# haoy945/DeMF

Hardware: AMD Instinct MI355X
Metric: DeMF fusion fwd+bwd scenes/sec at 20k pts + 530x730 RGB (higher is better)
Workload: dtype f32; 1 GPU; BASELINE configs[2]: full DeMF fusion hot path fwd+loss+bwd+allreduce+AdamW, 8 scenes/GPU x (20000 pts, 800x1120 -> 4-level 256-ch pyramid), 256 queries, H=8 L=4 P=2, fp32; compute_mode=f32, scenes_per_gpu=8, parallelism=dp1, cloud=uniform

## Files before the change

### demf_amd/_ffi.py

```python
import ctypes
import os

_HERE = os.path.dirname(os.path.abspath(__file__))
LIB_PATH = os.environ.get("DEMF_LIB_PATH") or os.path.join(_HERE, "lib", "libdemf_hip.so")

_c_int = ctypes.c_int
_c_float = ctypes.c_float
_ptr = ctypes.c_void_p

SIGNATURES = {
    "demf_stream_create_cu_masked": [_ptr, _c_int, _c_int, _ptr],
    "demf_spin_us": [_c_int, _ptr],
    "demf_conv_nhwc_f32": [_c_int] * 9 + [_ptr, _ptr, _c_int, _ptr, _ptr, _c_int, _c_int, _ptr, _ptr],
    "demf_conv_stem7_nhwc4_f32": [_c_int] * 4 + [_ptr, _ptr, _c_int, _ptr, _c_int, _ptr, _ptr],
    "demf_maxpool3x3s2_nhwc_f32": [_c_int] * 4 + [_ptr, _ptr, _ptr],
    "demf_nchw3_to_nhwc4_f32": [_c_int] * 3 + [_ptr, _ptr, _ptr],
    "demf_groupnorm_nhwc_f32": [_c_int] * 4 + [_c_float, _ptr, _ptr, _ptr, _ptr, _ptr, ctypes.c_longlong, _ptr],
    "demf_fps_f32": [_c_int, _c_int, _c_int, _ptr, _ptr, _ptr, _ptr],
    "demf_fps_ws_f32": [_c_int, _c_int, _c_int, _ptr, _ptr, ctypes.c_longlong, _ptr, _ptr],
    "demf_ball_query_f32": [_c_int, _c_int, _c_int, _c_float, _c_float, _c_int, _ptr, _ptr,
                            _ptr, _ptr],
    "demf_ball_query_grid_ws": [_c_int, _c_int, _ptr, _ptr],
    "demf_ball_query_grid_f32": [_c_int, _c_int, _c_int, _c_float, _c_int] + [_ptr] * 6,
    "demf_group_points_fwd": [_c_int] * 5 + [_ptr] * 4,
# ... 60 lines not shown
    "demf_multi_add": [_c_int, _ptr, _c_int, _ptr],
    "demf_multi_add_sumsq": [_c_int, _ptr, _c_int, _ptr, _ptr],
    "demf_scalars_accum": [_c_int, _ptr, _ptr, _c_float, _ptr],
    "demf_mlp_gemm_fwd": [_c_int] * 4 + [_ptr] * 6,
    "demf_mlp_gemm_fwd_pool": [_c_int] * 4 + [_ptr] * 5 + [_c_int] + [_ptr] * 5,
    "demf_mlp_gemm_fwd_bn": [_c_int] * 4 + [_ptr] * 7 + [_c_float, _c_float] + [_ptr] * 7,
    "demf_mlp_gemm_fwd_pool_bn": [_c_int] * 4 + [_ptr] * 5 + [_c_int] + [_ptr] * 6 + [_c_float, _c_float] + [_ptr] * 7,
    "demf_mlp_gemm_fwd_bn_st": [_c_int] * 4 + [_ptr] * 7 + [_c_float, _c_float] + [_ptr] * 6 + [_c_int, _ptr],
    "demf_mlp_gemm_fwd_pool_bn_st": [_c_int] * 4 + [_ptr] * 5 + [_c_int] + [_ptr] * 4 + [_c_float, _c_float] + [_ptr] * 6 + [_c_int, _ptr],
    "demf_pool_select": [_c_int] * 2 + [_ptr] * 9,
    "demf_pool_select_slot0": [_c_int] * 2 + [_ptr] * 7,
    "demf_mlp_first_stats": [_c_int] * 2 + [_ptr] * 5 + [_c_float, _c_float] + [_ptr] * 7,
    "demf_mlp_gemm_fwd_bn_x4": [_c_int] * 2 + [_ptr] * 8 + [_c_float, _c_float] + [_ptr] * 7,
    "demf_mlp_bwd_fused_x4": [_c_int] * 3 + [_ptr] * 11,
    "demf_mlp_bwd_pool": [_c_int] * 4 + [_ptr] * 17,
    "demf_mlp_bwd_pool_ws": [_c_int, _ptr],
    "demf_bn_finalize": [_c_int, ctypes.c_longlong] + [_ptr] * 3 + [_c_float, _c_float] + [_ptr] * 7,
    "demf_l2norm_rows_fwd": [_c_int] * 2 + [_ptr] * 4,
    "demf_l2norm_rows_bwd": [_c_int] * 2 + [_ptr] * 5,
    "demf_vote_combine_fwd": [_c_int] * 2 + [_ptr] * 7,
    "demf_vote_combine_bwd": [_c_int] * 2 + [_ptr] * 7,
    "demf_bnrelu_maxpool_fwd": [_c_int] * 3 + [_ptr] * 5,
    "demf_bn_bwd_reduce": [_c_int] * 3 + [_ptr] * 9,
    "demf_bn_bwd_vectors": [_c_int, ctypes.c_longlong] + [_ptr] * 8,
    "demf_mlp_gemm_bwd_dx": [_c_int] * 4 + [_ptr] * 3 + [_c_int] + [_ptr] * 5,
    "demf_mlp_gemm_bwd_dx_first": [_c_int] * 3 + [_ptr] * 10,
    "demf_mlp_first_finish": [_c_int, ctypes.c_longlong] + [_ptr] * 7,
    "demf_mlp_gemm_bwd_dx_red": [_c_int] * 4 + [_ptr] * 3 + [_c_int] + [_ptr] * 9,
    "demf_mlp_gemm_bwd_dx_w": [_c_int] * 4 + [_ptr] * 3 + [_c_int] + [_ptr] * 5,
    "demf_mlp_bwd_fused": [_c_int] * 3 + [_ptr] * 3 + [_c_int] + [_ptr] * 15 + [_c_int, _ptr],
    "demf_mlp_bwd_fused_cols": [_c_int] * 5 + [_ptr] * 3 + [_c_int] + [_ptr] * 14,
    "demf_mlp_bwd_fused_wide": [_c_int] * 3 + [_ptr] * 3 + [_c_int] + [_ptr] * 14,
    "demf_mlp_last_form": [],
    "demf_switch_at": [_c_int, _ptr, _ptr, _ptr],
    "demf_mlp_gemm_bwd_dx_red_v": [_c_int] * 4 + [_ptr] * 3 + [_c_int] + [_ptr] * 13,
    "demf_bn_bwd_reduce_vectors": [_c_int] * 3 + [_ptr] * 11 + [_c_int, _ptr],
    "demf_mlp_gemm_bwd_dw": [_c_int] * 4 + [_ptr] * 3 + [_c_int] + [_ptr] * 6,
    "demf_mlp_gemm_bwd_dw_ld": [_c_int] * 4 + [_ptr] * 3 + [_c_int] + [_ptr] * 5 + [_c_int, _ptr],
    "demf_head_loss_fwd": [_c_int] * 3 + [_ptr] * 14,
    "demf_head_loss_bwd": [_c_int] * 3 + [_ptr] * 17,
    "demf_ca_head_loss_fwd": [_c_int] * 3 + [_ptr] * 12,
    "demf_ca_head_loss_bwd": [_c_int] * 3 + [_ptr] * 16,
    "demf_vote_loss": [_c_int] * 4 + [_c_float] + [_ptr] * 10,
    "demf_vote_loss_fwd": [_c_int] * 4 + [_c_float] + [_ptr] * 8,
    "demf_msda_fwd_f32": [_c_int] * 7 + [_ptr] * 7,
    "demf_msda_bwd_f32": [_c_int] * 7 + [_ptr] * 10,
    "demf_msda_fwd_bf16": [_c_int] * 7 + [_ptr] * 7,
    "demf_msda_bwd_bf16": [_c_int] * 7 + [_ptr] * 10,
    "demf_gemm_f32": [_ptr, _ptr],
    "demf_gemm_group_f32": [_ptr, _c_int, _ptr],
    "demf_set_compute_dtype": [_c_int],
    "demf_set_f16_terms": [_c_int],
    "demf_get_compute_dtype": [],
    "demf_ctx_push": [_ptr],
    "demf_ctx_pop": [],
    "demf_gemm_f32_ctx": [_ptr] * 3,
    "demf_gemm_group_f32_ctx": [_ptr, _ptr, _c_int, _ptr],
    "demf_mlp_gemm_fwd_ctx": [_ptr] + [_c_int] * 4 + [_ptr] * 6,
    "demf_multi_copy": [_c_int, _ptr, _c_int, _ptr],
    "demf_zero_f32": [ctypes.c_longlong, _ptr, _ptr],
    "demf_add_dropout_ln_fwd": [_c_int] * 2 + [_ptr] * 4 + [_c_float] * 2 + [_ptr, _c_int] + [_ptr] * 4,
    "demf_add_dropout_ln_bwd": [_c_int] * 2 + [_ptr] * 5 + [_c_float, _ptr, _c_int, _ptr, _c_int] + [_ptr] * 4,
    "demf_attn_core_fwd": [_c_int] * 4 + [_ptr, _c_float, _c_float, _ptr, _c_int] + [_ptr] * 5,
    "demf_attn_core_bwd": [_c_int] * 4 + [_ptr] * 4 + [_c_float, _c_float, _ptr, _c_int] + [_ptr] * 2,
    "demf_softmax_dropout_fwd": [_c_int] * 2 + [_ptr, _c_float, _ptr, _c_int] + [_ptr] * 3,
    "demf_softmax_dropout_bwd": [_c_int] * 2 + [_ptr, _c_float, _ptr, _c_int] + [_ptr] * 2,
# ... 76 lines not shown
```

### demf_amd/csrc/mlp_bwd.hip

```cpp
#include "common.h"
#include "bn_fin.h"
#include "wide_map.h"

namespace demf {

using f32x16 = float __attribute__((ext_vector_type(16)));
using bf16x8 = __bf16 __attribute__((ext_vector_type(8)));
using bf16x4 = __bf16 __attribute__((ext_vector_type(4)));
using bf16x2 = __bf16 __attribute__((ext_vector_type(2)));

struct FusedBwdArgs {
  int R, N, K, ns;
  const float* Yl;
  const float* G;
  const float* dP;
  const int* arg;
  const float* vec;
  const float* Xp;
  const float* pss;
  const float* pmi;
  const float* W;
  float* dX;
  float* dW;
  double* g12;
  const float* fX;
  double* fsum;
  BnVecFin vfin;
  int ldk, ldw, fld, fc0;
  const float* W0;
  int dbg;
  int nchunk;
};

template <int P>
__device__ __forceinline__ void split_planes(float x, __bf16 (&o)[P]) {
  if constexpr (P == 2) {
    const _Float16 h = (_Float16)x;
    o[0] = __builtin_bit_cast(__bf16, h);
    o[1] = __builtin_bit_cast(__bf16, (_Float16)(x - (float)h));
    return;
  }
  o[0] = (__bf16)x;
  if constexpr (P == 3) {
    const float r = x - (float)o[0];
    o[1] = (__bf16)r;
    o[2] = (__bf16)(r - (float)o[1]);
  }
}

using f32x2 = float __attribute__((ext_vector_type(2)));
template <int P>
__device__ __forceinline__ void split_pair(float a, float b, unsigned (&o)[P]) {
  if constexpr (P == 2) {
    split2_f16(a, b, o[0], o[1]);
    return;
  }
  const f32x2 x = {a, b};
  const bf16x2 h = __builtin_convertvector(x, bf16x2);
  o[0] = __builtin_bit_cast(unsigned, h);
  if constexpr (P == 3) {
    const f32x2 r = x - __builtin_convertvector(h, f32x2);
    const bf16x2 m = __builtin_convertvector(r, bf16x2);
    o[1] = __builtin_bit_cast(unsigned, m);
    const f32x2 l = r - __builtin_convertvector(m, f32x2);
    o[2] = __builtin_bit_cast(unsigned, __builtin_convertvector(l, bf16x2));
// ... 19 lines not shown
    acc = __builtin_amdgcn_mfma_f32_32x32x16_bf16(a[0], b[0], acc, 0, 0, 0);
  } else {
    acc = __builtin_amdgcn_mfma_f32_32x32x16_bf16(a[0], b[0], acc, 0, 0, 0);
  }
}

__device__ __forceinline__ float f16_scale_for(float m) {
  int e = (int)((__builtin_bit_cast(unsigned, m) >> 23) & 0xff) - 127;
  e = 3 - e;
  e = e < -100 ? -100 : (e > 100 ? 100 : e);
  return __builtin_bit_cast(float, (unsigned)(e + 127) << 23);
}

template <int CW, bool B16>
__device__ __forceinline__ auto load_row(const float* __restrict__ base, size_t elem) {
  using vecT = float __attribute__((ext_vector_type(CW)));
  if constexpr (!B16) {
    return *reinterpret_cast<const vecT*>(base + elem);
  } else {
    const __bf16* b = reinterpret_cast<const __bf16*>(base) + elem;
    vecT v;
    if constexpr (CW == 4) {
      const uint2 u = *reinterpret_cast<const uint2*>(b);
      v[0] = __builtin_bit_cast(float, u.x << 16); v[1] = __builtin_bit_cast(float, u.x & 0xffff0000u);
      v[2] = __builtin_bit_cast(float, u.y << 16); v[3] = __builtin_bit_cast(float, u.y & 0xffff0000u);
    } else {
      const unsigned u = *reinterpret_cast<const unsigned*>(b);
      v[0] = __builtin_bit_cast(float, u << 16); v[1] = __builtin_bit_cast(float, u & 0xffff0000u);
    }
    return v;
  }
}

template <int NTN, int KT, int KG, bool SPARSE, int CM, int EPI, int ST = 0, bool WIDE = false>
__global__ __launch_bounds__(64 * NTN * KG, 512 / (64 * NTN * KG)) void mlp_bwd_fused_kernel(FusedBwdArgs p) {
  static_assert(!WIDE || (EPI == 0 && ST == 0), "WIDE: RED epilogue, fp32 rows");
  constexpr bool XB = (ST & 1) != 0, YB = (ST & 2) != 0;
  constexpr bool XR = (ST & 4) != 0;
  static_assert(!XR || (EPI == 1 && !XB), "recomputed rows: FIRST epilogue, no storage type");
  constexpr int P = CM == 2 ? 3 : (CM == 3 ? 2 : 1);
  constexpr bool H2 = CM == 3;
  constexpr int N = NTN * 32, K = KT * 32;
  constexpr int NW = NTN * KG;
  constexpr int NT = 64 * NW;
  constexpr int RS = 32;
  constexpr int KTW = KT / KG;
  constexpr int CW = 4 / KG;
  constexpr int LPB = 32 / CW;
  constexpr int QK = K / 4;
  constexpr int ER = NT / QK;
  constexpr int NH = NW / KT;
  constexpr int SL = NTN / NH;
  constexpr int CR = 16 / NH;
  static_assert(NW % KT == 0 && NH >= 1 && NTN % NH == 0 && SL >= 1, "dX wave map");
  static_assert(KG >= 1 && KTW >= 1 && KT % KG == 0 && (NW == 4 || NW == 8), "unsupported shape");
  static_assert(2 * ER == RS && 4 * (K / 64) == NW, "epilogue / staging maps");
  static_assert(EPI == 0 || (!SPARSE), "FIRST is a dense layer");
  constexpr int REGB = P * 2 * 2048;
  constexpr int XATB = P * K * 64;
  extern __shared__ __attribute__((aligned(16))) char smem[];
  char* s_reg = smem;
  char* s_xat = s_reg + NTN * REGB;
  float* s_dx = reinterpret_cast<float*>(s_xat + XATB);
  float* s_vy = s_dx + RS * K;
  float* s_px = s_vy + 5 * N;
  float* s_w0 = s_px + 4 * K;
  float* s_mx = s_w0 + 4 * K;
  const int tid = threadIdx.x, lane = tid & 63;
  const int wave = __builtin_amdgcn_readfirstlane(tid >> 6);
  const int lr = lane & 31, lh = lane >> 5;
  const int nt = wave % NTN, kg = wave / NTN;
  int w_fc0 = 0, w_slab0 = 0, w_step = 0;
  if constexpr (WIDE) {
    const WideBlock wb = wide_block((int)blockIdx.x, p.nchunk, (int)gridDim.x / p.nchunk);
    w_fc0 = __builtin_amdgcn_readfirstlane(wb.chunk * (KT * 32));
// ... 310 lines not shown
          }
          if constexpr (EPI == 0) {
            if constexpr (YB) {
              unsigned o0[1], o1[1];
              split_pair<1>(dx.x, dx.y, o0);
              split_pair<1>(dx.z, dx.w, o1);
              *reinterpret_cast<uint2*>(reinterpret_cast<__bf16*>(p.dX) + (size_t)row * p.ldk + 4 * e_cq) = make_uint2(o0[0], o1[0]);
            } else {
              *reinterpret_cast<float4*>(FB_PTR(p.dX) + (size_t)row * p.ldk + 4 * e_cq) = dx;
            }
          } else {
            const float4 x = *reinterpret_cast<const float4*>(p.fX + (size_t)row * 4);
            const float yv[4] = {y.x, y.y, y.z, y.w};
#pragma unroll
            for (int c = 0; c < 4; ++c) {
              fs[c][0] = __builtin_fmaf(dz[c], x.x, fs[c][0]);
              fs[c][1] = __builtin_fmaf(dz[c], x.y, fs[c][1]);
              fs[c][2] = __builtin_fmaf(dz[c], x.z, fs[c][2]);
              fs[c][3] = __builtin_fmaf(dz[c], x.w, fs[c][3]);
              fs[c][4] = __builtin_fmaf(yv[c], x.x, fs[c][4]);
              fs[c][5] = __builtin_fmaf(yv[c], x.y, fs[c][5]);
              fs[c][6] = __builtin_fmaf(yv[c], x.z, fs[c][6]);
              fs[c][7] = __builtin_fmaf(yv[c], x.w, fs[c][7]);
            }
            if (e_cq == 0) { fcx[0] += x.x; fcx[1] += x.y; fcx[2] += x.z; fcx[3] += x.w; }
          }
        }
      }
    }
  }

  __syncthreads();
  float* s_red = reinterpret_cast<float*>(smem);
  if (!(p.dbg & 1)) {
    const float inv = H2 ? 1.0f / sc_cur : 1.0f;
#pragma unroll
    for (int kk = 0; kk < KTW; ++kk)
#pragma unroll
      for (int r = 0; r < 16; ++r) {
        const int n = 32 * nt + (r & 3) + 8 * (r >> 2) + 4 * lh;
        const int k = 32 * (kg * KTW + kk) + lr;
        atomicAdd(FB_PTR(p.dW) + (size_t)n * p.ldw + k, H2 ? dwacc[kk][r] * inv : dwacc[kk][r]);
      }
  }
  constexpr int NV = EPI == 1 ? 8 + 32 + 4 : 8;
  float v[NV];
#pragma unroll
  for (int c = 0; c < 4; ++c) { v[c] = es1[c]; v[4 + c] = es2[c]; }
  if constexpr (EPI == 1) {
#pragma unroll
    for (int c = 0; c < 4; ++c)
#pragma unroll
      for (int q = 0; q < 8; ++q) v[8 + c * 8 + q] = fs[c][q];
#pragma unroll
    for (int c = 0; c < 4; ++c) v[40 + c] = fcx[c];
  }
#pragma unroll
  for (int i = 0; i < NV; ++i)
#pragma unroll
    for (int m = QK; m < 64; m <<= 1) v[i] += __shfl_xor(v[i], m);
  if (lane < QK) {
#pragma unroll
    for (int i = 0; i < NV; ++i) s_red[(wave * QK + lane) * NV + i] = v[i];
  }
  __syncthreads();
  for (int i = tid; i < QK * NV; i += NT) {
    const int cq = i / NV, q = i % NV;
    float t = 0.f;
#pragma unroll
    for (int w = 0; w < NW; ++w) t += s_red[(w * QK + cq) * NV + q];
    if (q < 8) {
      const int col = 4 * cq + (q & 3);
      if constexpr (EPI == 0) atomicAdd(p.g12 + (q >> 2) * p.fld + FB_FC0 + col, (double)t);
      else atomicAdd(p.fsum + (q >> 2) * K + col, (double)t);
    } else if (q < 40) {
      const int c = (q - 8) >> 3, s = (q - 8) & 7, col = 4 * cq + c;
      atomicAdd(p.fsum + (s < 4 ? 2 * K + col * 4 + s : 6 * K + col * 4 + (s - 4)), (double)t);
    } else if (cq == 0) {
      atomicAdd(p.fsum + 10 * K + (q - 40), (double)t);
    }
  }
  if constexpr (EPI == 0) {
    if (p.vfin.ticket != nullptr) {
      __shared__ int s_last;
      sync_drained();
      if (tid == 0) s_last = last_workgroup(p.vfin.ticket, (int)gridDim.x, (int)blockIdx.x);
      __syncthreads();
      if (s_last) bn_vec_finalize(p.vfin, p.fld, WIDE ? 0 : p.fc0, WIDE ? p.fld : K, p.g12, tid, NT);
    }
  }
#undef FB_FC0
#undef FB_STEP
#undef FB_PTR
}

struct PoolBwdArgs {
  int R, ns;
  const float* Xp;
  const float* pss;
  const float* pmi;
  const float* W;
  const float* vec;
  const float* dP;
  const int* arg;
  const float* yraw;
  float* dX;
  float* part;
  double* g12;
  BnVecFin vfin;
  int dbg;
};
constexpr int PB_N = 128, PB_K = 64, PB_RS = 64;
constexpr int PB_NACC = PB_N * PB_K;
constexpr int PB_LDA = PB_K + 4;
constexpr int PB_LDM = PB_K + 4;
// ... 356 lines not shown
    __shared__ int s_last;
    sync_drained();
    if (tid == 0) s_last = last_workgroup(p.vfin.ticket, (int)gridDim.x, (int)blockIdx.x);
    __syncthreads();
    if (s_last) bn_vec_finalize(p.vfin, K, 0, K, p.g12, tid, NT);
  }
}

__global__ __launch_bounds__(256) void pool_bwd_finish_k(int nslots, const float* __restrict__ part,
                                                         float* __restrict__ dW) {
  __shared__ float s_f[8][32];
  const int el = threadIdx.x & 31, sl = threadIdx.x >> 5;
  const int e = blockIdx.x * 32 + el;
  float t[8] = {0.f, 0.f, 0.f, 0.f, 0.f, 0.f, 0.f, 0.f};
  if (e < PB_NACC) {
    int s = sl;
    for (; s + 56 < nslots; s += 64) {
#pragma unroll
      for (int u = 0; u < 8; ++u) t[u] += part[(size_t)(s + 8 * u) * PB_NACC + e];
    }
    for (; s < nslots; s += 8) t[0] += part[(size_t)s * PB_NACC + e];
  }
  s_f[sl][el] = ((t[0] + t[1]) + (t[2] + t[3])) + ((t[4] + t[5]) + (t[6] + t[7]));
  __syncthreads();
  if (sl == 0 && e < PB_NACC)
    dW[e] = ((s_f[0][el] + s_f[1][el]) + (s_f[2][el] + s_f[3][el])) + ((s_f[4][el] + s_f[5][el]) + (s_f[6][el] + s_f[7][el]));
}

static int vectors_without_ticket(const BnVecFin& vf, int K, double* g12, demf_stream_t stream) {
  if (vf.gamma == nullptr || vf.ticket != nullptr) return DEMF_OK;
  return demf_bn_bwd_vectors(K, (long long)vf.count, g12, vf.gamma, vf.ss, vf.mi, vf.vec, vf.dgamma, vf.dbeta, stream);
}

template <int NTN, int KT, int KG, bool SPARSE, int CM, int EPI, int ST = 0, bool WIDE = false>
static int launch_fused(const FusedBwdArgs& a, hipStream_t s) {
  constexpr int P = CM == 2 ? 3 : (CM == 3 ? 2 : 1);
  constexpr int N = NTN * 32, K = KT * 32, NW = NTN * KG;
  const size_t bytes = (size_t)NTN * P * 2 * 2048 + (size_t)P * K * 64 + sizeof(float) * (32 * K + 5 * N + 4 * K + 4 * K + 24);
  static unsigned long long reserved = 0;
  if (!reserve_lds(reinterpret_cast<const void*>(&mlp_bwd_fused_kernel<NTN, KT, KG, SPARSE, CM, EPI, ST, WIDE>), (int)bytes,
                   &reserved)) {
    set_error("mlp_bwd_fused: cannot reserve %zu bytes of LDS", bytes);
    return DEMF_ELAUNCH;
  }
  const int nslab = (a.R + 31) / 32;
  const int cap = sw().persist_cus_bwd * (8 / NW);
  const int gx = WIDE ? a.nchunk * wide_members(nslab, a.nchunk, cap) : (nslab < cap ? nslab : cap);
  hipLaunchKernelGGL((mlp_bwd_fused_kernel<NTN, KT, KG, SPARSE, CM, EPI, ST, WIDE>), dim3(gx), dim3(64 * NW), bytes, s, a);
  return check_launch("mlp_bwd_fused");
}

}

using namespace demf;

static int fused_h2_mode() {
  return sw().f16_terms_bwd;
}
static bool fused_h2_on() { return fused_h2_mode() != 0; }

static int fused_supported(int R, int N, int K, int ns, int sparse, int first) {
  const int cm = compute_mode();
  if (cm != 1 && cm != 2) return 0;
  if (R < 1) return 0;
  if (sparse && (ns < 4 || ns % 4 != 0 || R % ns != 0)) return 0;
  if (first) return (N == 64 && K == 64 && !sparse) ? 1 : 0;
  return ((N == 128 && K == 64) || (N == 128 && K == 128) || (N == 64 && K == 64) || (N == 256 && K == 128)) ? 1 : 0;
}

extern "C" int demf_mlp_bwd_fused(int R, int N, int K, const float* G, const float* dP, const int* arg,
                                  int ns, const float* Y, const float* vec6, const float* W,
                                  const float* Yprev, const float* scale_shift_prev,
                                  const float* mean_invstd_prev, float* dX, float* dW, double* g12_prev,
                                  const float* X0, double* first_sums, const float* gamma_prev,
                                  float* vec6_prev, float* dgamma_prev, float* dbeta_prev,
                                  int store_flags, demf_stream_t stream) {
  const bool sparse = G == nullptr, first = first_sums != nullptr;
  DEMF_REQUIRE(fused_supported(R, N, K, ns, sparse, first),
               "mlp_bwd_fused: unsupported shape / mode R=%d N=%d K=%d ns=%d sparse=%d first=%d mode=%d",
               R, N, K, ns, (int)sparse, (int)first, compute_mode());
  DEMF_REQUIRE(Y && vec6 && W && Yprev && scale_shift_prev && mean_invstd_prev && dW &&
                   (G || (dP && arg)) && (first ? (X0 != nullptr) : (dX && g12_prev)),
// ... 84 lines not shown
  const bool sparse = G == nullptr;
  constexpr int Kc = 128;
  DEMF_REQUIRE(N == 256 && fused_supported(R, N, Kc, ns, sparse, 0) && Ktot > Kc && Ktot % Kc == 0 && Ktot <= 512,
               "mlp_bwd_fused_wide: unsupported shape / mode R=%d N=%d Ktot=%d ns=%d sparse=%d mode=%d",
               R, N, Ktot, ns, (int)sparse, compute_mode());
  DEMF_REQUIRE(Y && vec6 && W && Yprev && scale_shift_prev && mean_invstd_prev && dW && (G || (dP && arg)) && dX &&
                   g12_prev, "mlp_bwd_fused_wide: null pointer");
  set_last_form(DEMF_FORM_FUSED_WIDE);
  FusedBwdArgs a{};
  a.dbg = sw().bwd_dbg;
  a.R = R; a.N = N; a.K = Kc; a.ns = ns; a.Yl = Y; a.G = G; a.dP = dP; a.arg = arg; a.vec = vec6;
  a.Xp = Yprev; a.dX = dX; a.W = W; a.dW = dW;
  a.pss = scale_shift_prev; a.pmi = mean_invstd_prev; a.g12 = g12_prev;
  a.ldk = Ktot; a.ldw = Ktot; a.fld = Ktot; a.fc0 = 0; a.nchunk = Ktot / Kc;
  if (gamma_prev != nullptr) {
    DEMF_REQUIRE(vec6_prev && dgamma_prev && dbeta_prev, "mlp_bwd_fused_wide: vectors of layer l-1 need all three outputs");
    a.vfin = BnVecFin{(double)R, gamma_prev, scale_shift_prev, mean_invstd_prev, vec6_prev, dgamma_prev,
                      dbeta_prev, sched_slot()};
  }
  hipStream_t s = (hipStream_t)stream;
  const int cm = compute_mode();
  const bool h2 = f16_terms() && fused_h2_on();
  int rc;
  if (sparse) {
    rc = cm == 1 ? launch_fused<8, 4, 1, true, 1, 0, 0, true>(a, s)
                 : (h2 ? launch_fused<8, 4, 1, true, 3, 0, 0, true>(a, s) : launch_fused<8, 4, 1, true, 2, 0, 0, true>(a, s));
  } else {
    rc = cm == 1 ? launch_fused<8, 4, 1, false, 1, 0, 0, true>(a, s)
                 : (h2 ? launch_fused<8, 4, 1, false, 3, 0, 0, true>(a, s) : launch_fused<8, 4, 1, false, 2, 0, 0, true>(a, s));
  }
  return rc ? rc : vectors_without_ticket(a.vfin, Ktot, g12_prev, stream);
}

static int pool_bwd_grid(int R) {
  const int cus = sw().persist_cus_bwd;
  const int nslab = R / PB_RS;
  return nslab < cus ? (nslab > 0 ? nslab : 1) : cus;
}

extern "C" int demf_mlp_bwd_pool_ws(int R, long long* floats) {
  DEMF_REQUIRE(R >= 0 && floats, "mlp_bwd_pool_ws: bad arguments");
  *floats = (long long)pool_bwd_grid(R) * PB_NACC;
  return DEMF_OK;
}

extern "C" int demf_mlp_bwd_pool(int R, int N, int K, int ns, const float* dP, const int* arg,
                                 const float* yraw, const float* vec6, const float* W, const float* Yprev,
                                 const float* scale_shift_prev, const float* mean_invstd_prev, float* dX,
                                 float* dW, double* g12_prev, const float* gamma_prev, float* vec6_prev,
                                 float* dgamma_prev, float* dbeta_prev, float* workspace,
                                 demf_stream_t stream) {
  const int cm = compute_mode();
  DEMF_REQUIRE((cm == 1 || cm == 2) && N == PB_N && K == PB_K && ns == PB_RS && R >= ns && R % ns == 0,
               "mlp_bwd_pool: unsupported shape / mode R=%d N=%d K=%d ns=%d mode=%d", R, N, K, ns, cm);
  DEMF_REQUIRE(dP && arg && yraw && vec6 && W && Yprev && scale_shift_prev && mean_invstd_prev && dX && dW &&
                   g12_prev && workspace, "mlp_bwd_pool: null pointer");
  set_last_form(DEMF_FORM_POOL);
  PoolBwdArgs a{};
  a.R = R; a.ns = ns; a.Xp = Yprev; a.pss = scale_shift_prev; a.pmi = mean_invstd_prev; a.W = W; a.vec = vec6;
  a.dP = dP; a.arg = arg; a.yraw = yraw; a.dX = dX; a.part = workspace; a.g12 = g12_prev;
  a.dbg = sw().pb_dbg;
  if (gamma_prev != nullptr) {
    DEMF_REQUIRE(vec6_prev && dgamma_prev && dbeta_prev, "mlp_bwd_pool: vectors of layer l-1 need all three outputs");
    a.vfin = BnVecFin{(double)R, gamma_prev, scale_shift_prev, mean_invstd_prev, vec6_prev, dgamma_prev,
                      dbeta_prev, sched_slot()};
  }
// ... 49 lines not shown
```

### demf_amd/csrc/switches.h

```cpp
#pragma once

namespace demf {

#define DEMF_SWITCHES(X) \
  X(f32_native,         "DEMF_F32_NATIVE",         0,     "initial compute mode: 1 = fp32 MFMA (mode 0) instead of three bf16 terms (mode 2)") \
  X(f16_terms,          "DEMF_F16_TERMS",          1,     "initial two-fp16-term setting of mode 2 (demf_set_f16_terms overrides)") \
  X(f16_terms_bwd,      "DEMF_F16_TERMS_BWD",      1,     "fused backward: 0 = three bf16 terms, 1 = two fp16 terms, 2 = also the pool form") \
  X(x3_mask,            "DEMF_X3_MASK",            7,     "mode 2 per kernel family: bit 0 forward, bit 1 dX, bit 2 weight gradient") \
  X(static_tiles,       "DEMF_STATIC_TILES",       0,     "1 = static tile schedule, no BN-finalize ticket in the GEMM") \
  X(acc_repl,           "DEMF_ACC_REPL",           1,     "replicated statistics accumulators") \
  X(acc_repl_fwd,       "DEMF_ACC_REPL_FWD",       0,     "replicated accumulators in the forward finalize") \
  X(acc_repl_red,       "DEMF_ACC_REPL_RED",       0,     "replicated accumulators in the dX reduce finalize") \
  X(gemm_grid,          "DEMF_GEMM_GRID",          512,   "block cap of the persistent shared-MLP GEMM") \
  X(persist_cus,        "DEMF_PERSIST_CUS",        240,   "blocks of the weight-resident / producer-consumer forwards") \
  X(persist_cus_bwd,    "DEMF_PERSIST_CUS_BWD",    240,   "blocks of the fused backwards; unset = DEMF_PERSIST_CUS (reported value is the effective one)") \
  X(fwd_pc,             "DEMF_FWD_PC",             1,     "producer/consumer forward (K = 128)") \
  X(fwd_pc_min_r,       "DEMF_FWD_PC_MIN_R",       16384, "fewest rows for the producer/consumer forward") \
  X(fwd_res,            "DEMF_FWD_RES",            1,     "weight-resident forward (K = 64, N = 64 / 128)") \
  X(fwd_tile,           "DEMF_FWD_TILE",           1,     "few-row tile forward") \
  X(fwd_tile_max_r,     "DEMF_FWD_TILE_MAX_R",     16384, "most rows for the tile forward") \
  X(dx_tile,            "DEMF_DX_TILE",            1,     "few-row tile dX") \
  X(dx_tile_max_r,      "DEMF_DX_TILE_MAX_R",      16384, "most rows for the tile dX") \
  X(dx_chunks,          "DEMF_DX_CHUNKS",          0,     "chunked dX reduce") \
  X(pool_halves,        "DEMF_POOL_HALVES",        0,     "1 = ns 64 pooling on two co-scheduled column halves") \
  X(pool_dyn,           "DEMF_POOL_DYN",           1,     "dynamic tile schedule in the pooling GEMM") \
  X(x3_wide_split,      "DEMF_X3_WIDE_SPLIT",      1,     "0 = wide three-term forwards on the fp32 MFMA instead of a column split") \
  X(split_target,       "DEMF_SPLIT_TARGET",       256,   "blocks the column split aims at") \
  X(no_fin,             "DEMF_NO_FIN",             0,     "1 = no in-kernel BN finalize") \
  X(bnred_ns1_dense,    "DEMF_BNRED_NS1_DENSE",    1,     "dense form of the BN-backward reduce at ns = 1") \
  X(bnred_pooled_dense, "DEMF_BNRED_POOLED_DENSE", 1,     "dense form of the BN-backward reduce on pooled rows") \
  X(bnred_rpb,          "DEMF_BNRED_RPB",          8,     "rows per thread of the replicated dense reduce") \
  X(bnred_grid,         "DEMF_BNRED_GRID",         -1,    "block cap of the dense reduce; -1 = 1024 replicated, 256 otherwise") \
  X(bnred_rev,          "DEMF_BNRED_REV",          1,     "dense reduce visits its rows last to first") \
  X(bnred_sparse_rpt,   "DEMF_BNRED_SPARSE_RPT",   8,     "rows per thread of the sparse reduce") \
  X(bnred_sparse_grid,  "DEMF_BNRED_SPARSE_GRID",  1024,  "block cap of the sparse reduce") \
  X(dw_small_r,         "DEMF_DW_SMALL_R",         65536, "weight-gradient launches of at most this many rows use 64 x 64 sub-blocks") \
  X(dw_tile,            "DEMF_DW_TILE",            0,     "weight-gradient sub-block: 12 = 64 x 128, 21 = 128 x 64, 22, 11") \
  X(dw_f32,             "DEMF_DW_F32",             0,     "bf16 mode: weight gradient on fp32 operands") \
  X(dw_grid,            "DEMF_DW_GRID",            512,   "blocks of the grouped weight-gradient launch") \
  X(dw_dyn,             "DEMF_DW_DYN",             0,     "dynamic schedule of the weight-gradient launch") \
  X(dw_dbg,             "DEMF_DW_DBG",             0,     "weight gradient: phase-skip timing experiments") \
  X(dw_trace,           "DEMF_DW_TRACE",           0,     "print the step's weight-gradient products (tools/dw_micro.py)") \
  X(bwd_dbg,            "DEMF_BWD_DBG",            0,     "fused backward: phase-skip timing experiments") \
  X(pb_dbg,             "DEMF_PB_DBG",             0,     "pool backward: phase-skip timing experiments") \
  X(gemm_small_tiles,   "DEMF_GEMM_SMALL_TILES",   1024,  "demf_gemm_f32 launches of at most this many 64 x 64 tiles use the 32 x 32 kernel") \
  X(gemm_tn3,           "DEMF_GEMM_TN3",           1,     "0 = no three-term TN GEMM") \
  X(gemm_tn_split,      "DEMF_GEMM_TN_SPLIT",      0,     "forced K split of the TN GEMM") \
  X(tn_dbg,             "DEMF_TN_DBG",             0,     "TN GEMM: phase-skip timing experiments") \
  X(ln_bwd_blocks,      "DEMF_LN_BWD_BLOCKS",      256,   "blocks of the LayerNorm backward (at least 1)") \
  X(rg_dbg,             "DEMF_RG_DBG",             0,     "row GEMM chain: phase-skip timing experiments") \
  X(rg_ln128,           "DEMF_RG_LN128",           0,     "row GEMM chain: the 128-row LayerNorm form") \
  X(rg_waves8,          "DEMF_RG_WAVES8",          0,     "row GEMM chain: the 8-wave forms") \
  X(rg_add4,            "DEMF_RG_ADD4",            0,     "row GEMM chain: the adding form on 4 waves") \
  X(rg_one,             "DEMF_RG_ONE",             0,     "row GEMM chain: non-zero = one workgroup per CU") \
  X(conv_stream64,      "DEMF_CONV_STREAM64",      1,     "streaming 1x1 convolution at K = 64") \
  X(conv_streamk,       "DEMF_CONV_STREAMK",       3,     "streaming 1x1 convolution: bit 0 K = 128, bit 1 K = 256") \
  X(conv_stream_min,    "DEMF_CONV_STREAM_MIN",    16384, "fewest rows for the streaming convolution") \
  X(conv_wg3,           "DEMF_CONV_WG3",           0,     "three-plane convolutions: three workgroups per CU") \
  X(msda_head_wgs,      "DEMF_MSDA_HEAD_WGS",      256,   "workgroups the (scene, head)-major attention aims at") \
  X(msda_raw_lanes,     "DEMF_MSDA_RAW_LANES",     0,     "non-zero = 8 lanes per query in the raw form") \
  X(msda_xcd,           "DEMF_MSDA_XCD",           0,     "XCD-aware block order") \
  X(msda_nt,            "DEMF_MSDA_NT",            1,     "non-temporal loads of the raw offsets / logits") \
  X(gf_fwd_blocks,      "DEMF_GF_FWD_BLOCKS",      1024,  "block cap of the group-first forward") \
  X(gf_bwd_blocks,      "DEMF_GF_BWD_BLOCKS",      0,     "block cap of the group-first backward (0 = its own choice)") \
  X(gf_fin,             "DEMF_GF_FIN",             1,     "0 = group-first forward without the in-kernel finalize") \
  X(gf_recompute,       "DEMF_GF_RECOMPUTE",       1,     "0 = group-first backward reads stored activations") \
  X(gf_wacc,            "DEMF_GF_WACC",            1,     "0 = group-first backward without the in-kernel weight gradient") \
  X(colsum_rows,        "DEMF_COLSUM_ROWS",        64,    "fewest rows per block of the column sum") \
  X(invert_split,       "DEMF_INVERT_SPLIT",       1,     "invert_index as five launches when the lists leave LDS; 2 = from 32 768 entries, 0 = never") \
  X(three_nn_split,     "DEMF_THREE_NN_SPLIT",     1,     "split form of three_nn") \
  X(fps_check_split,    "DEMF_FPS_CHECK_SPLIT",    1,     "two-kernel form of the FPS order check") \
  X(fps_prune,          "DEMF_FPS_PRUNE",          1,     "box-pruned FPS on large clouds") \
  X(fps_pair,           "DEMF_FPS_PAIR",           -1,    "per-pair cached maxima: -1 = above 16 slots per lane, 0 / 1 force") \
  X(fps_pair_waves,     "DEMF_FPS_PAIR_WAVES",     16,    "waves of the pair kernel (8 or 16)") \
  X(fps_waves,          "DEMF_FPS_WAVES",          16,    "waves of the pruned kernel (8 or 16)")

// ... 10 lines not shown
```

### demf_amd/csrc/wide_map.h

```cpp
#pragma once

#if defined(__HIPCC__)
#define DEMF_WM_HD __host__ __device__ __forceinline__
#else
#define DEMF_WM_HD static inline
#endif

namespace demf {

struct WideBlock {
  int chunk;
  int first;
  int stride;
};

DEMF_WM_HD int wide_members(int nslab, int nchunk, int cap) {
  int g = cap / nchunk;
  if (g > nslab) g = nslab;
  if (g < 1) g = 1;
  if (g >= 8) g -= g % 8;
  return g;
}

DEMF_WM_HD int wide_run(int gpc) { return gpc >= 8 ? 8 : gpc; }

DEMF_WM_HD WideBlock wide_block(int block, int nchunk, int gpc) {
  const int rw = wide_run(gpc);
  const int run = block / (rw * nchunk), within = block % (rw * nchunk);
  WideBlock b;
  b.chunk = within / rw;
  b.first = run * rw + within % rw;
  b.stride = gpc;
  return b;
}

}
```

### include/demf_hip.h

```cpp
#ifndef DEMF_HIP_H_
#define DEMF_HIP_H_

#include <stdint.h>

#ifdef __cplusplus
extern "C" {
#endif

typedef void* demf_stream_t;

#define DEMF_OK 0
#define DEMF_EINVAL (-1)
#define DEMF_ELAUNCH (-2)
#define DEMF_EUNSUPPORTED (-3)

#define DEMF_ABI_VERSION 2

#define DEMF_INTERNAL

int demf_version(void);
const char* demf_last_error(void);

DEMF_INTERNAL int demf_stream_create_cu_masked(const int* cus, int n, int invert, void** out);

// ... 207 lines not shown
                                 int ns, float* pmax, int* amax, const float* gamma, const float* beta,
                                 float eps, float momentum, float* running_mean, float* running_var,
                                 long long* num_batches_tracked, float* scale_shift, float* mean_invstd,
                                 const float* conv_bias, int store_flags, demf_stream_t stream);

DEMF_INTERNAL int demf_mlp_bwd_fused(int R, int N, int K, const float* G, const float* dP, const int* arg, int ns,
                       const float* Y, const float* vec6, const float* W, const float* Yprev,
                       const float* scale_shift_prev, const float* mean_invstd_prev, float* dX,
                       float* dW, double* g12_prev, const float* X0, double* first_sums,
                       const float* gamma_prev, float* vec6_prev, float* dgamma_prev, float* dbeta_prev,
                       int store_flags, demf_stream_t stream);
DEMF_INTERNAL int demf_mlp_bwd_fused_cols(int R, int N, int Ktot, int c0, int Kc, const float* G, const float* dP,
                            const int* arg, int ns, const float* Y, const float* vec6, const float* W,
                            const float* Yprev, const float* scale_shift_prev,
                            const float* mean_invstd_prev, float* dX, float* dW, double* g12_prev,
                            const float* gamma_prev, float* vec6_prev, float* dgamma_prev,
                            float* dbeta_prev, demf_stream_t stream);
DEMF_INTERNAL int demf_mlp_bwd_fused_wide(int R, int N, int Ktot, const float* G, const float* dP, const int* arg, int ns,
                            const float* Y, const float* vec6, const float* W, const float* Yprev,
                            const float* scale_shift_prev, const float* mean_invstd_prev, float* dX,
                            float* dW, double* g12_prev, const float* gamma_prev, float* vec6_prev,
                            float* dgamma_prev, float* dbeta_prev, demf_stream_t stream);

#define DEMF_FORM_NONE 0
#define DEMF_FORM_GENERIC 1
#define DEMF_FORM_TILE 2
#define DEMF_FORM_RES 3
#define DEMF_FORM_PC 4
#define DEMF_FORM_FUSED 5
#define DEMF_FORM_FUSED_COLS 6
#define DEMF_FORM_FUSED_WIDE 7
#define DEMF_FORM_POOL 8
DEMF_INTERNAL int demf_mlp_last_form(void);

DEMF_INTERNAL int demf_switch_at(int index, const char** name, int* value, int* dflt);

DEMF_INTERNAL int demf_mlp_first_stats(int R, int N0, const float* X, const float* W0, double* moments, const float* gamma,
                         const float* beta, float eps, float momentum, float* running_mean,
                         float* running_var, long long* num_batches_tracked, float* scale_shift,
                         float* mean_invstd, const float* conv_bias, demf_stream_t stream);
DEMF_INTERNAL int demf_mlp_gemm_fwd_bn_x4(int R, int N, const float* X4, const float* W0, const float* prev_scale_shift,
                            const float* Wt, float* Y, double* stats, const float* gamma, const float* beta,
                            float eps, float momentum, float* running_mean, float* running_var,
                            long long* num_batches_tracked, float* scale_shift, float* mean_invstd,
                            const float* conv_bias, demf_stream_t stream);
DEMF_INTERNAL int demf_mlp_bwd_fused_x4(int R, int N, int K, const float* G, const float* Y, const float* vec6,
                          const float* W, const float* X0, const float* W0, const float* scale_shift_prev,
                          const float* mean_invstd_prev, float* dW, double* first_sums, demf_stream_t stream);

DEMF_INTERNAL int demf_mlp_bwd_pool_ws(int R, long long* floats);
DEMF_INTERNAL int demf_mlp_bwd_pool(int R, int N, int K, int ns, const float* dP, const int* arg, const float* yraw,
                      const float* vec6, const float* W, const float* Yprev,
                      const float* scale_shift_prev, const float* mean_invstd_prev, float* dX, float* dW,
                      double* g12_prev, const float* gamma_prev, float* vec6_prev, float* dgamma_prev,
                      float* dbeta_prev, float* workspace, demf_stream_t stream);

DEMF_INTERNAL int demf_mlp_gemm_bwd_dw(int R, int N, int K, int ldx, const float* G, const float* dP,
                         const int* arg, int ns, const float* Y, const float* vec6,
                         const float* Xprev, const float* prev_scale_shift, float* dW,
                         demf_stream_t stream);
DEMF_INTERNAL int demf_mlp_gemm_bwd_dw_ld(int R, int N, int K, int ldx, const float* G, const float* dP,
                            const int* arg, int ns, const float* Y, const float* vec6,
                            const float* Xprev, const float* prev_scale_shift, float* dW, int lddw,
                            demf_stream_t stream);

typedef struct demf_dw_job {
// ... 312 lines not shown
```

Measured before the change: 1926 scenes/s.

## Fold fused-backward dW partials per same-XCD workgroup group before atomics

For fused MLP backward kernels with 128 input channels, each workgroup writes its dW partial tile to a global slot buffer. A per-group ticket picks the last-arriving workgroup of a group of (by default) 4 same-XCD workgroups, which sums the partials and issues the atomicAdds alone. This cuts global float atomics on dW by roughly the group size, at the cost of extra global stores and loads, release/acquire fences and a serial reduction tail in one workgroup per group. It also adds a switch and a debug query for ticket state.

```diff
diff --git a/demf_amd/_ffi.py b/demf_amd/_ffi.py
--- a/demf_amd/_ffi.py
+++ b/demf_amd/_ffi.py
@@ -116,6 +116,7 @@
     "demf_mlp_bwd_fused_cols": [_c_int] * 5 + [_ptr] * 3 + [_c_int] + [_ptr] * 14,
     "demf_mlp_bwd_fused_wide": [_c_int] * 3 + [_ptr] * 3 + [_c_int] + [_ptr] * 14,
     "demf_mlp_last_form": [],
+    "demf_mlp_bwd_flush_state": [_ptr, _ptr],
     "demf_switch_at": [_c_int, _ptr, _ptr, _ptr],
     "demf_mlp_gemm_bwd_dx_red_v": [_c_int] * 4 + [_ptr] * 3 + [_c_int] + [_ptr] * 13,
     "demf_bn_bwd_reduce_vectors": [_c_int] * 3 + [_ptr] * 11 + [_c_int, _ptr],
diff --git a/demf_amd/csrc/mlp_bwd.hip b/demf_amd/csrc/mlp_bwd.hip
--- a/demf_amd/csrc/mlp_bwd.hip
+++ b/demf_amd/csrc/mlp_bwd.hip
@@ -30,7 +30,12 @@
   const float* W0;
   int dbg;
   int nchunk;
+  int fgroup;
 };
+
+constexpr int FLUSH_SLOTS = 256, FLUSH_SLOT = 256 * 128, FLUSH_TICKETS = 256;
+__device__ float g_flush_slots[(size_t)FLUSH_SLOTS * FLUSH_SLOT];
+__device__ int g_flush_tickets[FLUSH_TICKETS];
 
 template <int P>
 __device__ __forceinline__ void split_planes(float x, __bf16 (&o)[P]) {
@@ -116,7 +121,7 @@
   }
 }
 
-template <int NTN, int KT, int KG, bool SPARSE, int CM, int EPI, int ST = 0, bool WIDE = false>
+template <int NTN, int KT, int KG, bool SPARSE, int CM, int EPI, int ST = 0, bool WIDE = false, bool FL = false>
 __global__ __launch_bounds__(64 * NTN * KG, 512 / (64 * NTN * KG)) void mlp_bwd_fused_kernel(FusedBwdArgs p) {
   static_assert(!WIDE || (EPI == 0 && ST == 0), "WIDE: RED epilogue, fp32 rows");
   constexpr bool XB = (ST & 1) != 0, YB = (ST & 2) != 0;
@@ -125,6 +130,7 @@
   constexpr int P = CM == 2 ? 3 : (CM == 3 ? 2 : 1);
   constexpr bool H2 = CM == 3;
   constexpr int N = NTN * 32, K = KT * 32;
+  static_assert(!FL || (EPI == 0 && ST == 0 && K == 128), "FL: RED epilogue, fp32 rows, 128 input channels");
   constexpr int NW = NTN * KG;
   constexpr int NT = 64 * NW;
   constexpr int RS = 32;
@@ -501,16 +507,59 @@
 
   __syncthreads();
   float* s_red = reinterpret_cast<float*>(smem);
-  if (!(p.dbg & 1)) {
-    const float inv = H2 ? 1.0f / sc_cur : 1.0f;
+  [[maybe_unused]] int fl_v = (int)blockIdx.x, fl_n = 0, fl_ch = 0;
+  [[maybe_unused]] FlushGroup fl_g{0, 1, 0};
+  [[maybe_unused]] float4* fl_slot0 = nullptr;
+  [[maybe_unused]] auto flush_add = [&]() {
 #pragma unroll
     for (int kk = 0; kk < KTW; ++kk)
 #pragma unroll
       for (int r = 0; r < 16; ++r) {
         const int n = 32 * nt + (r & 3) + 8 * (r >> 2) + 4 * lh;
         const int k = 32 * (kg * KTW + kk) + lr;
-        atomicAdd(FB_PTR(p.dW) + (size_t)n * p.ldw + k, H2 ? dwacc[kk][r] * inv : dwacc[kk][r]);
-      }
+        atomicAdd(FB_PTR(p.dW) + (size_t)n * p.ldw + k, dwacc[kk][r]);
+      }
+  };
+  if constexpr (!FL) {
+    if (!(p.dbg & 1)) {
+      const float inv = H2 ? 1.0f / sc_cur : 1.0f;
+#pragma unroll
+      for (int kk = 0; kk < KTW; ++kk)
+#pragma unroll
+        for (int r = 0; r < 16; ++r) {
+          const int n = 32 * nt + (r & 3) + 8 * (r >> 2) + 4 * lh;
+          const int k = 32 * (kg * KTW + kk) + lr;
+          atomicAdd(FB_PTR(p.dW) + (size_t)n * p.ldw + k, H2 ? dwacc[kk][r] * inv : dwacc[kk][r]);
+        }
+    }
+  } else if (!(p.dbg & 1)) {
+    if constexpr (H2) {
+      const float inv = 1.0f / sc_cur;
+#pragma unroll
+      for (int kk = 0; kk < KTW; ++kk)
+#pragma unroll
+        for (int r = 0; r < 16; ++r) dwacc[kk][r] *= inv;
+    }
+    fl_n = (int)gridDim.x;
+    if constexpr (WIDE) {
+      fl_n = (int)gridDim.x / p.nchunk;
+      const WideBlock wb = wide_block((int)blockIdx.x, p.nchunk, fl_n);
+      fl_v = wide_member(wb);
+      fl_ch = wb.chunk;
+    }
+    fl_g = flush_group(fl_v, fl_n, p.fgroup);
+    fl_slot0 = reinterpret_cast<float4*>(g_flush_slots) + (size_t)(fl_ch * fl_n) * (FLUSH_SLOT / 4) +
+               (size_t)(wave * KTW * 4) * 64 + lane;
+    if (fl_g.size > 1) {
+      float4* mine = fl_slot0 + (size_t)fl_v * (FLUSH_SLOT / 4);
+#pragma unroll
+      for (int kk = 0; kk < KTW; ++kk)
+#pragma unroll
+        for (int q = 0; q < 4; ++q)
+          mine[(kk * 4 + q) * 64] = make_float4(dwacc[kk][4 * q], dwacc[kk][4 * q + 1], dwacc[kk][4 * q + 2], dwacc[kk][4 * q + 3]);
+    } else {
+      flush_add();
+    }
   }
   constexpr int NV = EPI == 1 ? 8 + 32 + 4 : 8;
   float v[NV];
@@ -549,7 +598,63 @@
       atomicAdd(p.fsum + 10 * K + (q - 40), (double)t);
     }
   }
-  if constexpr (EPI == 0) {
+  if constexpr (FL) {
+    int* s_flag = reinterpret_cast<int*>(s_mx + 16);
+    const bool grouped = !(p.dbg & 1) && fl_g.size > 1;
+    sync_drained();
+    if (tid == 0) {
+      int last = 0;
+      if (grouped) {
+        if (!(p.dbg & 8)) __builtin_amdgcn_fence(__ATOMIC_RELEASE, "agent");
+        drain_vmem();
+        int* t = g_flush_tickets + fl_ch * flush_tickets(fl_n, p.fgroup) + fl_g.ticket;
+        last = __hip_atomic_fetch_add(t, 1, __ATOMIC_RELAXED, __HIP_MEMORY_SCOPE_AGENT) == fl_g.size - 1;
+        if (last) {
+          atomicExch(t, 0);
+          __builtin_amdgcn_fence(__ATOMIC_ACQUIRE, "agent");
+          drain_vmem();
+        }
+      }
+      s_flag[0] = last;
+      s_flag[1] = p.vfin.ticket != nullptr ? last_workgroup(p.vfin.ticket, (int)gridDim.x, (int)blockIdx.x) : 0;
+    }
+    __syncthreads();
+    if (__builtin_amdgcn_readfirstlane(s_flag[0])) {
+      if (!(p.dbg & 4)) {
+        for (int i = 0; i < fl_g.size; i += 2) {
+          const int va = fl_g.first + 8 * i, vb = va + 8;
+          const bool ona = va != fl_v, onb = i + 1 < fl_g.size && vb != fl_v;
+          const float4* sa = fl_slot0 + (size_t)va * (FLUSH_SLOT / 4);
+          const float4* sb = fl_slot0 + (size_t)vb * (FLUSH_SLOT / 4);
+          float4 ta[KTW * 4], tb[KTW * 4];
+          if (ona) {
+#pragma unroll
+            for (int e = 0; e < KTW * 4; ++e) ta[e] = sa[e * 64];
+          }
+          if (onb) {
+#pragma unroll
+            for (int e = 0; e < KTW * 4; ++e) tb[e] = sb[e * 64];
+          }
+          if (ona) {
+#pragma unroll
+            for (int e = 0; e < KTW * 4; ++e) {
+              dwacc[e / 4][4 * (e % 4)] += ta[e].x; dwacc[e / 4][4 * (e % 4) + 1] += ta[e].y;
+              dwacc[e / 4][4 * (e % 4) + 2] += ta[e].z; dwacc[e / 4][4 * (e % 4) + 3] += ta[e].w;
+            }
+          }
+          if (onb) {
+#pragma unroll
+            for (int e = 0; e < KTW * 4; ++e) {
+              dwacc[e / 4][4 * (e % 4)] += tb[e].x; dwacc[e / 4][4 * (e % 4) + 1] += tb[e].y;
+              dwacc[e / 4][4 * (e % 4) + 2] += tb[e].z; dwacc[e / 4][4 * (e % 4) + 3] += tb[e].w;
+            }
+          }
+        }
+      }
+      if (!(p.dbg & 2)) flush_add();
+    }
+    if (s_flag[1]) bn_vec_finalize(p.vfin, p.fld, WIDE ? 0 : p.fc0, WIDE ? p.fld : K, p.g12, tid, NT);
+  } else if constexpr (EPI == 0) {
     if (p.vfin.ticket != nullptr) {
       __shared__ int s_last;
       sync_drained();
@@ -972,22 +1077,42 @@
   return demf_bn_bwd_vectors(K, (long long)vf.count, g12, vf.gamma, vf.ss, vf.mi, vf.vec, vf.dgamma, vf.dbeta, stream);
 }
 
+template <int NTN, int KT, int KG, bool SPARSE, int CM, int EPI, int ST, bool WIDE, bool FL>
+static int launch_fused_variant(const FusedBwdArgs& a, int gx, size_t bytes, hipStream_t s) {
+  static unsigned long long reserved = 0;
+  if (!reserve_lds(reinterpret_cast<const void*>(&mlp_bwd_fused_kernel<NTN, KT, KG, SPARSE, CM, EPI, ST, WIDE, FL>), (int)bytes,
+                   &reserved)) {
+    set_error("mlp_bwd_fused: cannot reserve %zu bytes of LDS", bytes);
+    return DEMF_ELAUNCH;
+  }
+  hipLaunchKernelGGL((mlp_bwd_fused_kernel<NTN, KT, KG, SPARSE, CM, EPI, ST, WIDE, FL>), dim3(gx), dim3(64 * (NTN * KG)), bytes, s, a);
+  return check_launch("mlp_bwd_fused");
+}
+
+constexpr int FLUSH_GROUP_DEFAULT = 4, FLUSH_MAX_SLABS_DEFAULT = 16;
+static int g_flush_launches = 0;
+
 template <int NTN, int KT, int KG, bool SPARSE, int CM, int EPI, int ST = 0, bool WIDE = false>
 static int launch_fused(const FusedBwdArgs& a, hipStream_t s) {
   constexpr int P = CM == 2 ? 3 : (CM == 3 ? 2 : 1);
   constexpr int N = NTN * 32, K = KT * 32, NW = NTN * KG;
   const size_t bytes = (size_t)NTN * P * 2 * 2048 + (size_t)P * K * 64 + sizeof(float) * (32 * K + 5 * N + 4 * K + 4 * K + 24);
-  static unsigned long long reserved = 0;
-  if (!reserve_lds(reinterpret_cast<const void*>(&mlp_bwd_fused_kernel<NTN, KT, KG, SPARSE, CM, EPI, ST, WIDE>), (int)bytes,
-                   &reserved)) {
-    set_error("mlp_bwd_fused: cannot reserve %zu bytes of LDS", bytes);
-    return DEMF_ELAUNCH;
-  }
   const int nslab = (a.R + 31) / 32;
   const int cap = sw().persist_cus_bwd * (8 / NW);
   const int gx = WIDE ? a.nchunk * wide_members(nslab, a.nchunk, cap) : (nslab < cap ? nslab : cap);
-  hipLaunchKernelGGL((mlp_bwd_fused_kernel<NTN, KT, KG, SPARSE, CM, EPI, ST, WIDE>), dim3(gx), dim3(64 * NW), bytes, s, a);
-  return check_launch("mlp_bwd_fused");
+  if constexpr (EPI == 0 && ST == 0 && K == 128) {
+    const bool own = sw().bwd_flush_group < 0;
+    const int G = own ? FLUSH_GROUP_DEFAULT : sw().bwd_flush_group;
+    const int fn = WIDE ? gx / a.nchunk : gx;
+    if (G > 1 && (!own || nslab <= FLUSH_MAX_SLABS_DEFAULT * fn) && !sw().static_tiles && gx >= 2 * G && gx <= FLUSH_SLOTS &&
+        (WIDE ? a.nchunk : 1) * flush_tickets(fn, G) <= FLUSH_TICKETS) {
+      FusedBwdArgs b = a;
+      b.fgroup = G;
+      __atomic_fetch_add(&g_flush_launches, 1, __ATOMIC_RELAXED);
+      return launch_fused_variant<NTN, KT, KG, SPARSE, CM, EPI, ST, WIDE, true>(b, gx, bytes, s);
+    }
+  }
+  return launch_fused_variant<NTN, KT, KG, SPARSE, CM, EPI, ST, WIDE, false>(a, gx, bytes, s);
 }
 
 }
@@ -1138,6 +1263,21 @@
   return rc ? rc : vectors_without_ticket(a.vfin, Ktot, g12_prev, stream);
 }
 
+extern "C" int demf_mlp_bwd_flush_state(int* busy_tickets, int* launches) {
+  DEMF_REQUIRE(busy_tickets && launches, "mlp_bwd_flush_state: null pointer");
+  int host[FLUSH_TICKETS];
+  if (hipDeviceSynchronize() != hipSuccess ||
+      hipMemcpyFromSymbol(host, HIP_SYMBOL(g_flush_tickets), sizeof(host), 0, hipMemcpyDeviceToHost) != hipSuccess) {
+    set_error("mlp_bwd_flush_state: %s", hipGetErrorString(hipGetLastError()));
+    return DEMF_ELAUNCH;
+  }
+  int busy = 0;
+  for (int i = 0; i < FLUSH_TICKETS; ++i) busy += host[i] != 0;
+  *busy_tickets = busy;
+  *launches = __atomic_load_n(&g_flush_launches, __ATOMIC_RELAXED);
+  return DEMF_OK;
+}
+
 static int pool_bwd_grid(int R) {
   const int cus = sw().persist_cus_bwd;
   const int nslab = R / PB_RS;
diff --git a/demf_amd/csrc/switches.h b/demf_amd/csrc/switches.h
--- a/demf_amd/csrc/switches.h
+++ b/demf_amd/csrc/switches.h
@@ -42,6 +42,7 @@
   X(dw_dbg,             "DEMF_DW_DBG",             0,     "weight gradient: phase-skip timing experiments") \
   X(dw_trace,           "DEMF_DW_TRACE",           0,     "print the step's weight-gradient products (tools/dw_micro.py)") \
   X(bwd_dbg,            "DEMF_BWD_DBG",            0,     "fused backward: phase-skip timing experiments") \
+  X(bwd_flush_group,    "DEMF_BWD_FLUSH_GROUP",    -1,    "fused backward, 128 input channels: dW partials folded per group of this many workgroups of one XCD before the atomics; 0 = every workgroup adds its own, -1 = per kernel form") \
   X(pb_dbg,             "DEMF_PB_DBG",             0,     "pool backward: phase-skip timing experiments") \
   X(gemm_small_tiles,   "DEMF_GEMM_SMALL_TILES",   1024,  "demf_gemm_f32 launches of at most this many 64 x 64 tiles use the 32 x 32 kernel") \
   X(gemm_tn3,           "DEMF_GEMM_TN3",           1,     "0 = no three-term TN GEMM") \
diff --git a/demf_amd/csrc/wide_map.h b/demf_amd/csrc/wide_map.h
--- a/demf_amd/csrc/wide_map.h
+++ b/demf_amd/csrc/wide_map.h
@@ -34,4 +34,25 @@
   return b;
 }
 
+struct FlushGroup {
+  int ticket;
+  int size;
+  int first;
+};
+
+DEMF_WM_HD int flush_tickets(int n, int G) { return 8 * (((n + 7) / 8 + G - 1) / G); }
+
+DEMF_WM_HD FlushGroup flush_group(int v, int n, int G) {
+  const int x = v % 8, j = v / 8;
+  const int cnt = n / 8 + (x < n % 8 ? 1 : 0);
+  const int g = j / G;
+  FlushGroup f;
+  f.ticket = x * (((n + 7) / 8 + G - 1) / G) + g;
+  f.size = cnt - g * G < G ? cnt - g * G : G;
+  f.first = x + 8 * g * G;
+  return f;
 }
+
+DEMF_WM_HD int wide_member(const WideBlock& b) { return b.first; }
+
+}
diff --git a/include/demf_hip.h b/include/demf_hip.h
--- a/include/demf_hip.h
+++ b/include/demf_hip.h
@@ -263,6 +263,7 @@
 #define DEMF_FORM_FUSED_WIDE 7
 #define DEMF_FORM_POOL 8
 DEMF_INTERNAL int demf_mlp_last_form(void);
+DEMF_INTERNAL int demf_mlp_bwd_flush_state(int* busy_tickets, int* launches);
 
 DEMF_INTERNAL int demf_switch_at(int index, const char** name, int* value, int* dflt);
 
```

New measurement: 1938 scenes/s, median of 6. About the same (+0.6%).
